# skipperro/selkies-gstreamer

Hardware: AMD Instinct MI355X
Metric: encoded fps + glass-to-glass p50 ms at 1920x1080; concurrent 60fps sessions/node (higher is better)
Workload: dtype uint8 pixels / int32 integer transforms (bit-exact vs CPU reference); 1 GPU; model=H.264 Constrained Baseline CAVLC, striped stripes 64px, CRF 25, global_batch=8, seq_len=1, parallelism=session-parallel dp1 x 8 sessions/GPU, resolution=1920x1080, backend=hip, deblock=auto, me_full=True, upload_overlap=False, frames_in_flight=1, num_refs=1, numa_node_rank0=0

## Files before the change

csrc/kernels/h264_kernels.hip:

```cpp
#include "h264_gpu.h"
#include "../codec/color.h"
#include "../codec/h264_mb.h"
#include "../codec/h264_ep.h"

namespace sk {
namespace h264 {
namespace gpu {

__device__ __forceinline__ int lane_id() { return threadIdx.x & 63; }

__device__ __forceinline__ void wave_sync() {
    __builtin_amdgcn_fence(__ATOMIC_RELEASE, "wavefront");
    __builtin_amdgcn_wave_barrier();
    __builtin_amdgcn_fence(__ATOMIC_ACQUIRE, "wavefront");
}

__device__ __forceinline__ int wave_sum(int v) {
    v += __builtin_amdgcn_mov_dpp(v, 0xB1, 0xF, 0xF, false);
    v += __builtin_amdgcn_mov_dpp(v, 0x4E, 0xF, 0xF, false);
    v += __builtin_amdgcn_mov_dpp(v, 0x124, 0xF, 0xF, false);
    v += __builtin_amdgcn_mov_dpp(v, 0x128, 0xF, 0xF, false);
    return __builtin_amdgcn_readlane(v, 0) + __builtin_amdgcn_readlane(v, 16) +
           __builtin_amdgcn_readlane(v, 32) + __builtin_amdgcn_readlane(v, 48);
}
// ... 212 lines not shown
            const uint4 a0 = *reinterpret_cast<const uint4*>(r0 + 4 * x0);
            const uint4 a1 = *reinterpret_cast<const uint4*>(r0 + 4 * x0 + 16);
            const uint4 b0 = *reinterpret_cast<const uint4*>(r1 + 4 * x0);
            const uint4 b1 = *reinterpret_cast<const uint4*>(r1 + 4 * x0 + 16);
            p0[0] = a0.x; p0[1] = a0.y; p0[2] = a0.z; p0[3] = a0.w;
            p0[4] = a1.x; p0[5] = a1.y; p0[6] = a1.z; p0[7] = a1.w;
            p1[0] = b0.x; p1[1] = b0.y; p1[2] = b0.z; p1[3] = b0.w;
            p1[4] = b1.x; p1[5] = b1.y; p1[6] = b1.z; p1[7] = b1.w;
        } else {
#pragma unroll
            for (int i = 0; i < 8; i++) {
                p0[i] = bgrx_px(r0, x0 + i, a.W);
                p1[i] = bgrx_px(r1, x0 + i, a.W);
            }
        }
        {
            const OverlayParams o0 = a.ov[0], o1 = a.ov[1];
            if (o0.on | o1.on) {
                const OverlayParams op[kOverlaySlots] = {o0, o1};
#pragma unroll
                for (int i = 0; i < 8; i++) {
                    const int x = sk_min(x0 + i, a.W - 1);
                    p0[i] = overlay_px(p0[i], x, y0, op, a.ov_img);
                    p1[i] = overlay_px(p1[i], x, y1, op, a.ov_img);
                }
            }
        }
        uint32_t ya[2] = {0, 0}, yb[2] = {0, 0}, cbw = 0, crw = 0;
#pragma unroll
        for (int q = 0; q < 4; q++) {
            uint8_t y[4], cb, cr;
            bgrx_quad_to_yuv((const uint8_t*)&p0[2 * q], (const uint8_t*)&p0[2 * q + 1], (const uint8_t*)&p1[2 * q],
                             (const uint8_t*)&p1[2 * q + 1], a.full_range, y, &cb, &cr);
            const int sh = 16 * (q & 1);
            ya[q >> 1] |= (uint32_t)(y[0] | (y[1] << 8)) << sh;
            yb[q >> 1] |= (uint32_t)(y[2] | (y[3] << 8)) << sh;
            cbw |= (uint32_t)cb << (8 * q);
            crw |= (uint32_t)cr << (8 * q);
        }
        const size_t oy = (size_t)(2 * qy) * a.stride_y + x0;
        const size_t oc = (size_t)qy * a.stride_c + x0 / 2;
        const uint2 pa = *reinterpret_cast<const uint2*>(a.prev.y + oy);
        const uint2 pb = *reinterpret_cast<const uint2*>(a.prev.y + oy + a.stride_y);
        const uint32_t pu = *reinterpret_cast<const uint32_t*>(a.prev.u + oc);
        const uint32_t pv = *reinterpret_cast<const uint32_t*>(a.prev.v + oc);
        diff = (pa.x != ya[0]) | (pa.y != ya[1]) | (pb.x != yb[0]) | (pb.y != yb[1]) | (pu != cbw) | (pv != crw);
        *reinterpret_cast<uint2*>(a.src.y + oy) = make_uint2(ya[0], ya[1]);
        *reinterpret_cast<uint2*>(a.src.y + oy + a.stride_y) = make_uint2(yb[0], yb[1]);
        *reinterpret_cast<uint32_t*>(a.src.u + oc) = cbw;
        *reinterpret_cast<uint32_t*>(a.src.v + oc) = crw;
    }
    if (diff || a.plan_ctl[1] == 0) mbd[item >> 1] = 1;
    __syncthreads();
    if (t < 16) {
        const int mbx = mbx0 + t;
        if (mbx < a.mb_w) a.mb_dirty[mby * a.mb_w + mbx] = (uint8_t)mbd[t];
    }
    if (__syncthreads_or(t < 16 && mbd[t] && mbx0 + t < a.mb_w) && t == 0)
        a.stripe_dirty[mby / a.rows_per_slice] = 1;
    host_words_store(a, host_words);
}

__global__ __launch_bounds__(256) void k_yuv_damage(FrameArgs a) {
    __shared__ int mbd[16];
    const int t = threadIdx.x;
    const int host_words = host_words_load(a);
    if (t < 16) mbd[t] = 0;
    __syncthreads();
    const int item = t & 31, qr = t >> 5;
    const int mby = blockIdx.y, mbx0 = blockIdx.x * 16;
    const int x0 = mbx0 * 16 + item * 8;
    const int qy = mby * 8 + qr;
    bool diff = false;
    if (x0 < a.stride_y) {
        const int W = a.W, H = a.H, cw = (W + 1) >> 1, ch = (H + 1) >> 1;
        const uint8_t* py = a.yuv;
        const uint8_t* pc = a.yuv + (size_t)W * H;
        const int y0 = min(2 * qy, H - 1), y1 = min(2 * qy + 1, H - 1), cy = min(qy, ch - 1);
        uint32_t ya[2] = {0, 0}, yb[2] = {0, 0}, cbw = 0, crw = 0;
#pragma unroll
        for (int i = 0; i < 8; i++) {
            const int x = min(x0 + i, W - 1);
            ya[i >> 2] |= (uint32_t)py[(size_t)y0 * W + x] << (8 * (i & 3));
            yb[i >> 2] |= (uint32_t)py[(size_t)y1 * W + x] << (8 * (i & 3));
        }
#pragma unroll
        for (int q = 0; q < 4; q++) {
            const int cx = min((x0 >> 1) + q, cw - 1);
            uint32_t u, v;
            if (a.yuv_fmt == 2) {
                const uint8_t* r = pc + (size_t)cy * (2 * cw) + 2 * cx;
                u = r[0];
                v = r[1];
            } else {
                u = pc[(size_t)cy * cw + cx];
                v = pc[(size_t)cw * ch + (size_t)cy * cw + cx];
            }
            cbw |= u << (8 * q);
            crw |= v << (8 * q);
        }
        const size_t oy = (size_t)(2 * qy) * a.stride_y + x0;
        const size_t oc = (size_t)qy * a.stride_c + x0 / 2;
        const uint2 pa = *reinterpret_cast<const uint2*>(a.prev.y + oy);
        const uint2 pb = *reinterpret_cast<const uint2*>(a.prev.y + oy + a.stride_y);
        const uint32_t pu = *reinterpret_cast<const uint32_t*>(a.prev.u + oc);
        const uint32_t pv = *reinterpret_cast<const uint32_t*>(a.prev.v + oc);
        diff = (pa.x != ya[0]) | (pa.y != ya[1]) | (pb.x != yb[0]) | (pb.y != yb[1]) | (pu != cbw) | (pv != crw);
        *reinterpret_cast<uint2*>(a.src.y + oy) = make_uint2(ya[0], ya[1]);
        *reinterpret_cast<uint2*>(a.src.y + oy + a.stride_y) = make_uint2(yb[0], yb[1]);
        *reinterpret_cast<uint32_t*>(a.src.u + oc) = cbw;
        *reinterpret_cast<uint32_t*>(a.src.v + oc) = crw;
    }
    if (diff || a.plan_ctl[1] == 0) mbd[item >> 1] = 1;
    __syncthreads();
    if (t < 16) {
        const int mbx = mbx0 + t;
        if (mbx < a.mb_w) a.mb_dirty[mby * a.mb_w + mbx] = (uint8_t)mbd[t];
    }
    if (__syncthreads_or(t < 16 && mbd[t] && mbx0 + t < a.mb_w) && t == 0)
        a.stripe_dirty[mby / a.rows_per_slice] = 1;
    host_words_store(a, host_words);
}

__device__ __forceinline__ uint32_t load_ref4(const uint8_t* row, int x, int stride) {
    if (x >= 0 && x + 3 <= stride - 1) {
        int xa = x & ~3, sh = x & 3;
        uint32_t w0 = *reinterpret_cast<const uint32_t*>(row + xa);
        if (sh == 0) return w0;
        uint32_t w1 = *reinterpret_cast<const uint32_t*>(row + xa + 4);
        return __builtin_amdgcn_alignbyte(w1, w0, sh);
    }
    uint32_t v = 0;
#pragma unroll
    for (int i = 0; i < 4; i++) v |= (uint32_t)row[sk_clip(x + i, 0, stride - 1)] << (8 * i);
    return v;
}

__device__ __forceinline__ uint32_t me_sad_lane(const FrameArgs& a, const uint8_t* refy, uint32_t sw, int mbx,
                                                int mby, int dx, int dy, int ylo, int yhi) {
    int l = lane_id();
    int row = l >> 2, col4 = (l & 3) * 4;
    int sy = sk_clip(mby * 16 + row + dy, ylo, yhi);
    uint32_t rw = load_ref4(refy + (size_t)sy * a.stride_y, mbx * 16 + col4 + dx, a.stride_y);
    return __builtin_amdgcn_sad_u8(sw, rw, 0u);
}

__device__ __forceinline__ int me_sad(const FrameArgs& a, const uint8_t* refy, uint32_t sw, int mbx,
                                      int mby, int dx, int dy, int ylo, int yhi) {
    return wave_sum((int)me_sad_lane(a, refy, sw, mbx, mby, dx, dy, ylo, yhi));
}

constexpr int kWin = 8;
constexpr int kWinWords = 10;
constexpr int kFsWinWords = kFsWin / 4 + 1;

struct MeWin {
    const uint32_t* w;
    int stride;
    int rad;
    int cx, cy;
    __device__ __forceinline__ bool has(int dx, int dy) const {
        return dx - cx >= -rad && dx - cx <= rad && dy - cy >= -rad && dy - cy <= rad;
    }
};

__device__ __forceinline__ uint32_t win_sad_lane(const MeWin& wn, uint32_t sw, int dx, int dy) {
    const int l = lane_id();
    const int row = l >> 2, col4 = (l & 3) * 4;
    const int bc = col4 + dx - wn.cx + wn.rad;
    const uint32_t* w = wn.w + (row + dy - wn.cy + wn.rad) * wn.stride + (bc >> 2);
    const int sh = bc & 3;
    const uint32_t rw = sh ? __builtin_amdgcn_alignbyte(w[1], w[0], sh) : w[0];
    return __builtin_amdgcn_sad_u8(sw, rw, 0u);
}

__device__ __forceinline__ int mb_activity(uint32_t sw) {
    const int psum = (int)(sw & 255) + (int)((sw >> 8) & 255) + (int)((sw >> 16) & 255) + (int)(sw >> 24);
    const int mean = (wave_sum(psum) + 128) >> 8;
    int dev = 0;
#pragma unroll
    for (int i = 0; i < 4; i++) dev += sk_abs((int)((sw >> (8 * i)) & 255) - mean);
    return wave_sum(dev);
}

__device__ __forceinline__ void me_search_mb(const FrameArgs& a, const SliceTask& t, const uint8_t* refy, int idx, int mbx,
                                             int mby, uint32_t sw, bool have_fs, int fsx, int fsy, uint32_t* win,
                                             bool big) {
    const int l = lane_id();
    if (t.action == ACT_I) {
        const int dev = mb_activity(sw);
        if (l == 0) a.me[idx] = MeResult{0, 0, 0, dev, 0, 0, 0};
        return;
    }
    const int ylo = t.pic_row0 * 16, yhi = (t.pic_row0 + t.pic_rows) * 16 - 1;
    const int lam = lambda_for_qp(rc_me_qp(*a.rc, t.qp));
    const int R = a.me_range;
    MeWin wn{win, big ? kFsWinWords : kWinWords, big ? kFsR : -1, 0, 0};
    auto sad_lane = [&](int dx, int dy) {
        return wn.has(dx, dy) ? win_sad_lane(wn, sw, dx, dy) : me_sad_lane(a, refy, sw, mbx, mby, dx, dy, ylo, yhi);
    };
    int cx[7], cy[7];
    bool ok[7];
    auto slot = [&](int k, bool valid, int ox, int oy) {
        const int j = valid ? oy * a.mb_w + ox : idx;
        ok[k] = valid;
        cx[k] = sk_clip(a.mvfield[2 * j], -R, R);
        cy[k] = sk_clip(a.mvfield[2 * j + 1], -R, R);
    };
    cx[0] = 0; cy[0] = 0; ok[0] = true;
    slot(1, true, mbx, mby);
    slot(2, mbx > 0, mbx - 1, mby);
    slot(3, mbx + 1 < a.mb_w, mbx + 1, mby);
    slot(4, mby - 1 >= t.pic_row0, mbx, mby - 1);
    slot(5, mby + 1 < t.pic_row0 + t.pic_rows, mbx, mby + 1);
    ok[6] = have_fs;
    cx[6] = sk_clip(fsx, -R, R);
    cy[6] = sk_clip(fsy, -R, R);
    int sd[8];
    {
        uint32_t p[8];
#pragma unroll
        for (int k = 0; k < 7; k++) p[k] = ok[k] ? sad_lane(cx[k], cy[k]) : 0u;
        p[7] = 0u;
#pragma unroll
        for (int k = 0; k < 8; k += 2) {
            const uint32_t s2 = (uint32_t)wave_sum((int)(p[k] | (p[k + 1] << 16)));
            sd[k] = (int)(s2 & 0xffff);
            sd[k + 1] = (int)(s2 >> 16);
        }
    }
    int bx = 0, by = 0;
    int bsad = sd[0];
    int bcost = bsad + lam * (sk_se_bits(0) + sk_se_bits(0));
#pragma unroll
    for (int k = 1; k < 7; k++) {
        if (!ok[k]) continue;
        int c = sd[k] + lam * (sk_se_bits(4 * cx[k]) + sk_se_bits(4 * cy[k]));
        if (c < bcost) { bcost = c; bx = cx[k]; by = cy[k]; bsad = sd[k]; }
    }
    if (!(big && wn.has(bx, by))) {
        wave_sync();
        const int r = l >> 1, h = l & 1;
        const int y = sk_clip(mby * 16 + by - kWin + r, ylo, yhi);
        const uint8_t* rowp = refy + (size_t)y * a.stride_y;
        const int x0 = mbx * 16 + bx - kWin + 16 * h;
#pragma unroll
        for (int k = 0; k < 5; k++) win[r * kWinWords + 4 * h + k] = load_ref4(rowp, x0 + 4 * k, a.stride_y);
        wn = MeWin{win, kWinWords, kWin, bx, by};
        wave_sync();
    }
    const int ddx[4] = {0, -1, 1, 0}, ddy[4] = {-1, 0, 0, 1};
    for (int it = 0; it < a.me_iters; it++) {
        uint32_t p[4];
        bool in_r[4];
#pragma unroll
        for (int k = 0; k < 4; k++) {
            const int x = bx + ddx[k], y = by + ddy[k];
            in_r[k] = !(x < -R || x > R || y < -R || y > R);
            p[k] = in_r[k] ? sad_lane(x, y) : 0u;
        }
        const uint32_t s01 = (uint32_t)wave_sum((int)(p[0] | (p[1] << 16)));
        const uint32_t s23 = (uint32_t)wave_sum((int)(p[2] | (p[3] << 16)));
        const int sds[4] = {(int)(s01 & 0xffff), (int)(s01 >> 16), (int)(s23 & 0xffff), (int)(s23 >> 16)};
        int nb = -1, ncost = bcost, nsad = 0;
#pragma unroll
        for (int k = 0; k < 4; k++) {
            if (!in_r[k]) continue;
            int x = bx + ddx[k], y = by + ddy[k];
            int c = sds[k] + lam * (sk_se_bits(4 * x) + sk_se_bits(4 * y));
            if (c < ncost) { ncost = c; nb = k; nsad = sds[k]; }
        }
        if (nb < 0) break;
        bx += ddx[nb]; by += ddy[nb]; bcost = ncost; bsad = nsad;
    }
    const int dev = mb_activity(sw);
    int refi = 0;
    if (t.num_refs > 1 && a.mb_dirty[idx]) {
        const int s1 = me_sad(a, ref1_planes(a, mby / a.rows_per_slice).y, sw, mbx, mby, 0, 0, ylo, yhi);
        if (s1 + 3 * lam < bcost) {
            bx = by = 0;
            bsad = s1;
            refi = 1;
        }
    }
    if (l == 0) {
        MeResult r;
        r.mvx = (int16_t)bx;
        r.mvy = (int16_t)by;
        r.sad = bsad;
        r.intra_est = dev;
        r.ref = (int16_t)refi;
        r.fx = r.fy = 0;
        a.me[idx] = r;
    }
}

__global__ __launch_bounds__(64) void k_motion_search(FrameArgs a) {
    __shared__ uint32_t win[32 * kWinWords];
    int nmb = a.mb_w * a.mb_h;
    int idx = xcd_remap(blockIdx.x, gridDim.x);
    if (idx >= nmb) return;
    int mbx = idx % a.mb_w, mby = idx / a.mb_w;
    const SliceTask t = a.tasks[mby / a.rows_per_slice];
    if (t.action != ACT_P && t.action != ACT_I) return;
    int l = lane_id();
    uint32_t sw = *reinterpret_cast<const uint32_t*>(a.src.y + (size_t)(mby * 16 + (l >> 2)) * a.stride_y +
                                                     mbx * 16 + (l & 3) * 4);
    const bool have_fs = a.me_full && t.action == ACT_P && a.mb_dirty[idx];
    const int fsx = have_fs ? a.fs_mv[2 * idx] : 0, fsy = have_fs ? a.fs_mv[2 * idx + 1] : 0;
    me_search_mb(a, t, ref0_planes(a, mby / a.rows_per_slice).y, idx, mbx, mby, sw, have_fs, fsx, fsy, win, false);
}

typedef int v4i __attribute__((ext_vector_type(4)));

constexpr int kFsBlkWords = 5;
constexpr int kFsSqInts = 2 * kFsR + 4;

__device__ __forceinline__ uint64_t fs_search(const FrameArgs& a, const uint8_t* refy, uint32_t* win, uint32_t* blk, int* sq,
                                              int mbx, int mby, uint32_t sw, int ylo, int yhi) {
    constexpr int WW = kFsWin / 4;
    constexpr int WP = kFsWinWords;
    constexpr int BP = kFsBlkWords;
    constexpr int SP = kFsSqInts;
    const int l = lane_id();
    for (int i = l; i < kFsWin * WW; i += 64) {
        const int wy = i / WW, q = i - wy * WW;
        const int y = sk_clip(mby * 16 - kFsR + wy, ylo, yhi);
        win[wy * WP + q] = load_ref4(refy + (size_t)y * a.stride_y, mbx * 16 - kFsR + 4 * q, a.stride_y);
    }
    blk[(l >> 2) * BP + (l & 3)] = sw;
    wave_sync();
    if (l < kFsWin) {
        uint32_t rw[WW];
#pragma unroll
        for (int q = 0; q < WW; q++) rw[q] = win[l * WP + q];
        int sqv[kFsWin];
#pragma unroll
        for (int c = 0; c < kFsWin; c++) {
            const int v = (int)((rw[c >> 2] >> (8 * (c & 3))) & 255) - 128;
            sqv[c] = v * v;
        }
        int acc = 0;
#pragma unroll
        for (int c = 0; c < 16; c++) acc += sqv[c];
        int out[2 * kFsR];
        out[0] = acc;
#pragma unroll
        for (int x = 1; x < 2 * kFsR; x++) {
            acc += sqv[x + 15] - sqv[x - 1];
            out[x] = acc;
        }
#pragma unroll
        for (int x = 0; x < 2 * kFsR; x += 4)
            *reinterpret_cast<int4*>(&sq[l * SP + x]) = make_int4(out[x], out[x + 1], out[x + 2], out[x + 3]);
    }
    wave_sync();
    if (l < 2 * kFsR) {
        int col[kFsWin];
#pragma unroll
        for (int r = 0; r < kFsWin; r++) col[r] = sq[r * SP + l];
        int acc = 0;
#pragma unroll
        for (int r = 0; r < 16; r++) acc += col[r];
#pragma unroll
        for (int dy = 0; dy < 2 * kFsR; dy++) {
            sq[dy * SP + l] = acc;
            acc += col[dy + 16] - col[dy];
        }
    }
    const int i16 = l & 15, g = l >> 4;
    v4i acc[2][2];
#pragma unroll
    for (int mt = 0; mt < 2; mt++)
#pragma unroll
        for (int nt = 0; nt < 2; nt++) acc[mt][nt] = v4i{0, 0, 0, 0};
#pragma unroll
    for (int ks = 0; ks < kFsWin / 4; ks++) {
        const int rr = 4 * ks + g;
        v4i bf[2];
#pragma unroll
        for (int nt = 0; nt < 2; nt++) {
            const int src = rr - (16 * nt + i16);
            const bool in = src >= 0 && src < 16;
#pragma unroll
            for (int q = 0; q < 4; q++) bf[nt][q] = in ? (int)(blk[(in ? src : 0) * BP + q] ^ 0x80808080u) : 0;
        }
#pragma unroll
        for (int mt = 0; mt < 2; mt++) {
            const int b0 = 16 * mt + i16;
            const uint32_t* wr = win + rr * WP + (b0 >> 2);
            const int sh = b0 & 3;
            uint32_t w5[5];
#pragma unroll
            for (int q = 0; q < 5; q++) w5[q] = wr[q];
            v4i af;
#pragma unroll
            for (int q = 0; q < 4; q++) af[q] = (int)(__builtin_amdgcn_alignbyte(w5[q + 1], w5[q], sh) ^ 0x80808080u);
#pragma unroll
            for (int nt = 0; nt < 2; nt++)
                if (ks >= 4 * nt && ks <= 4 * nt + 7)
                    acc[mt][nt] = __builtin_amdgcn_mfma_i32_16x16x64_i8(af, bf[nt], acc[mt][nt], 0, 0, 0);
        }
    }
    wave_sync();
    uint64_t best = ~0ull;
#pragma unroll
    for (int mt = 0; mt < 2; mt++)
#pragma unroll
        for (int nt = 0; nt < 2; nt++) {
            const int dyw = 16 * nt + i16;
            const int4 sv = *reinterpret_cast<const int4*>(&sq[dyw * SP + 16 * mt + 4 * g]);
            const int svr[4] = {sv.x, sv.y, sv.z, sv.w};
#pragma unroll
            for (int reg = 0; reg < 4; reg++) {
                const int dxw = 16 * mt + 4 * g + reg;
                const uint64_t k = fs_key(svr[reg] - 2 * acc[mt][nt][reg], dyw, dxw);
                best = k < best ? k : best;
            }
        }
#pragma unroll
    for (int o = 1; o < 64; o <<= 1) {
        const uint64_t other = __shfl_xor(best, o);
        best = other < best ? other : best;
    }
    return best;
}

__global__ __launch_bounds__(256) void k_me(FrameArgs a) {
    __shared__ uint32_t win_s[4][kFsWin * kFsWinWords];
    __shared__ uint32_t blk_s[4][16 * kFsBlkWords];
    __shared__ __align__(16) int sq_s[4][kFsWin * kFsSqInts];
    static_assert(kFsWin * kFsWinWords >= 32 * kWinWords, "the small window lives in the wave's win_s region");
    const int w = threadIdx.x >> 6, l = lane_id();
    const int nmb = a.mb_w * a.mb_h;
    const int idx = xcd_remap(blockIdx.x, gridDim.x) * 4 + w;
    if (idx >= nmb) return;
    const int mbx = idx % a.mb_w, mby = idx / a.mb_w;
    const SliceTask t = a.tasks[mby / a.rows_per_slice];
    if (t.action != ACT_P && t.action != ACT_I) return;
    const uint8_t* refy = ref0_planes(a, mby / a.rows_per_slice).y;
    const uint32_t sw = *reinterpret_cast<const uint32_t*>(a.src.y + (size_t)(mby * 16 + (l >> 2)) * a.stride_y +
                                                           mbx * 16 + (l & 3) * 4);
    bool have_fs = false, big = false;
    int fsx = 0, fsy = 0;
    if (t.action == ACT_P && a.mb_dirty[idx]) {
        have_fs = true;
        const int ylo = t.pic_row0 * 16, yhi = (t.pic_row0 + t.pic_rows) * 16 - 1;
        const int R = a.me_range;
        const int px = sk_clip(a.mvfield[2 * idx], -R, R), py = sk_clip(a.mvfield[2 * idx + 1], -R, R);
        if (me_sad(a, refy, sw, mbx, mby, px, py, ylo, yhi) == 0) {
            fsx = px;
            fsy = py;
        } else {
            const uint64_t best = fs_search(a, refy, win_s[w], blk_s[w], sq_s[w], mbx, mby, sw, ylo, yhi);
            fsx = __builtin_amdgcn_readfirstlane(fs_key_dx(best));
            fsy = __builtin_amdgcn_readfirstlane(fs_key_dy(best));
            big = true;
        }
        if (l == 0) {
            a.fs_mv[2 * idx] = (int16_t)fsx;
            a.fs_mv[2 * idx + 1] = (int16_t)fsy;
        }
    }
    me_search_mb(a, t, refy, idx, mbx, mby, sw, have_fs, fsx, fsy, win_s[w], big);
}

__global__ __launch_bounds__(256) void k_plan(FrameArgs a) {
    const int ns = a.num_slices, tid = threadIdx.x;
    StripeState* st = a.plan_state;
    StripeState& pic = st[ns];
    if (a.plan_ctl[1] == 1) {
        if (a.fullframe) {
            bool idr = true;
            for (int s = tid; s < ns; s += 256) idr &= a.tasks[s].final_action == ACT_I && a.tasks[s].idr_on_intra;
            idr = __syncthreads_and(idr);
            if (tid == 0) commit_picture(pic, idr, a.plan_cfg.num_refs);
            if (a.ltr_excl && tid == 0)
                ltr::ltr_commit_rps(a.ltr_slots, a.ltr_state[ns], idr, a.tasks[0].frame_num, a.mb_w * a.mb_h, 0, ns,
                                    a.ltr_task);
            else if (a.ltr_slots && tid == 0)
                ltr::ltr_commit(a.ltr_slots, a.ltr_state[ns], true, idr, a.tasks[0].frame_num, a.mb_w * a.mb_h, 0, ns,
                                a.ltr_task);
        } else {
            if (a.ltr_slots)
                for (int s = tid; s < ns; s += 256) {
                    const SliceTask& t = a.tasks[s];
                    ltr::ltr_commit(a.ltr_slots, a.ltr_state[s], t.final_action != ACT_NONE,
                                    t.final_action == ACT_I && t.idr_on_intra, t.frame_num, t.num_rows * a.mb_w, s, s + 1,
                                    a.ltr_task);
                }
            for (int s = tid; s < ns; s += 256)
                commit_stripe(st[s], a.tasks[s].final_action, a.plan_cfg.num_refs, a.tasks[s].idr_on_intra != 0);
        }
    }
    __shared__ int hk[6];
    if (tid < 6) hk[tid] = a.key_dev[tid];
    __syncthreads();
    const int kq = hk[0];
    const bool key = kq != a.plan_ctl[0];
    __syncthreads();
    if (key) {
        for (int s = tid; s < ns; s += 256) st[s].need_idr = true;
        if (tid == 0) pic.need_idr = true;
    }
    __syncthreads();
    PlanConfig pc = a.plan_cfg;
    const int qo = hk[1];
    const int po = hk[2];
    if (qo > 0) pc.qp = qo;
    if (po > 0) pc.paint_qp = po;
    {
        const int mode = hk[5] != a.rc->seq ? hk[3] : a.rc->mode;
        if (mode == RC_CBR) pc.use_paint_over = 0;
    }
    for (int s = tid; s < ns; s += 256) {
        st[s].subpel_prev = st[s].subpel_hits;
        st[s].subpel_hits = 0;
        const int r0 = s * a.rows_per_slice, nr = min(a.rows_per_slice, a.mb_h - r0);
        plan_stripe(pc, st[s], pic, a.stripe_dirty[s] != 0, r0, nr, a.mb_h, a.tasks[s]);
        a.stripe_dirty[s] = 0;
    }
    __syncthreads();
    if (tid == 0) {
        a.plan_ctl[0] = kq;
        a.plan_ctl[1] = 1;
    }
}

__global__ __launch_bounds__(256) void k_ltr_match(FrameArgs a) {
    __shared__ int red[4];
    const int band = blockIdx.x, c = blockIdx.y, s = blockIdx.z, tid = threadIdx.x;
    const int ns = a.num_slices;
    const SliceTask t = a.tasks[s];
    const int s0 = a.fullframe ? 0 : s, s1 = a.fullframe ? ns : s + 1;
    const int mb0 = (a.fullframe ? 0 : t.first_row) * a.mb_w, n = (a.fullframe ? a.mb_h : t.num_rows) * a.mb_w;
    int nd = 0, key = 0, anyp = 0;
    for (int i = tid; i < n; i += 256) nd += a.mb_dirty[mb0 + i] != 0;
    for (int i = s0 + tid; i < s1; i += 256) {
        key |= a.tasks[i].action == ACT_I;
        anyp |= a.tasks[i].action == ACT_P;
    }
    nd = wave_sum(nd);
    if (lane_id() == 0) red[tid >> 6] = nd;
    key = __syncthreads_or(key);
    anyp = __syncthreads_or(anyp);
    nd = red[0] + red[1] + red[2] + red[3];
    const int valid = a.ltr_state[a.fullframe ? ns : s].valid;
    const bool gate = anyp && !key && ltr::ltr_large(nd, n) && valid != 0;
    if (band == 0 && c == 0 && tid == 0) {
        a.ltr_cnt[2 * s] = nd;
        a.ltr_cnt[2 * s + 1] = gate;
    }
    if (!gate || t.action != ACT_P || band >= t.num_rows || (c > 0 && !((valid >> (c - 1)) & 1))) return;
    const uint8_t* ref = c ? a.ltr.y + (size_t)(c - 1) * a.ltr_ny : a.ref.y;
    const size_t o = (size_t)(t.first_row + band) * 16 * a.stride_y;
    const uint4* q = reinterpret_cast<const uint4*>(a.src.y + o);
    const uint4* r = reinterpret_cast<const uint4*>(ref + o);
    uint32_t sum = 0;
    for (int i = tid; i < a.stride_y; i += 256) {
        const uint4 x = q[i], y = r[i];
        sum = __builtin_amdgcn_sad_u8(x.x, y.x, sum);
        sum = __builtin_amdgcn_sad_u8(x.y, y.y, sum);
        sum = __builtin_amdgcn_sad_u8(x.z, y.z, sum);
        sum = __builtin_amdgcn_sad_u8(x.w, y.w, sum);
    }
    sum = (uint32_t)wave_sum((int)sum);
    __syncthreads();
    if (lane_id() == 0) red[tid >> 6] = (int)sum;
    __syncthreads();
    if (tid == 0)
        a.ltr_part[((size_t)s * ltr::kLtrSadCols + c) * a.rows_per_slice + band] =
            (uint32_t)red[0] + (uint32_t)red[1] + (uint32_t)red[2] + (uint32_t)red[3];
}

__global__ __launch_bounds__(256) void k_ltr_decide(FrameArgs a) {
    const int ns = a.num_slices, tid = threadIdx.x;
    for (int i = tid; i < ns * ltr::kLtrSadCols; i += 256) {
        const int s = i / ltr::kLtrSadCols, c = i - s * ltr::kLtrSadCols;
        const int valid = a.ltr_state[a.fullframe ? ns : s].valid;
        uint32_t sum = 0;
        if (a.ltr_cnt[2 * s + 1] && a.tasks[s].action == ACT_P && c <= a.ltr_slots && (c == 0 || ((valid >> (c - 1)) & 1)))
            for (int b = 0; b < a.tasks[s].num_rows; b++) sum += a.ltr_part[(size_t)i * a.rows_per_slice + b];
        a.ltr_sad[i] = sum;
    }
    __syncthreads();
    const int streams = a.fullframe ? 1 : ns;
    for (int k = tid; k < streams; k += 256) {
        const int s0 = a.fullframe ? 0 : k, s1 = a.fullframe ? ns : k + 1;
        bool key = false, anyp = false;
        int rows = 0;
        for (int s = s0; s < s1; s++) {
            key |= a.tasks[s].action == ACT_I;
            anyp |= a.tasks[s].action == ACT_P;
            rows += a.tasks[s].num_rows;
        }
        if (a.ltr_excl) ltr::ltr_expire(a.ltr_slots, a.ltr_state[ns], a.tasks[s0].frame_num, a.ltr_max_age);
        ltr::ltr_decide(a.ltr_slots, a.ltr_state[a.fullframe ? ns : k], a.ltr_cnt[2 * s0], rows * a.mb_w, anyp && !key,
                        a.tasks[s0].frame_num, kFrameNumMask, s0, s1,
                        [&](int s) { return a.tasks[s].action == ACT_P; }, a.ltr_sad, a.ltr_task);
        for (int s = s0; s < s1; s++)
            if (a.ltr_task[s].slot >= 0 && !a.ltr_excl) a.tasks[s].num_refs = 2;
    }
}

__global__ __launch_bounds__(256) void k_decide(FrameArgs a) {
    __shared__ long long red[2][4];
    const int s = blockIdx.x;
    SliceTask& t = a.tasks[s];
    const bool planned_p = t.action == ACT_P;
    const bool p = planned_p && t.allow_scenecut;
    __shared__ int red1[4];
    long long sad = 0, dev = 0;
    int ref1 = 0;
    if (planned_p || t.action == ACT_I) {
        const int first = t.first_row * a.mb_w, nmb = t.num_rows * a.mb_w;
        for (int i = threadIdx.x; i < nmb; i += 256) {
            const MeResult r = a.me[first + i];
// ... 2080 lines not shown
            w[2 + (le >> 1)] |= (uint32_t)bh << sh;
            w[10] |= (bv ? 1u << le : 0u) | (bh ? 16u << le : 0u);
        }
    const int qc = cur.qpy, cc = H264_CHROMA_QP[qc];
    w[4] = db_pack_par((left.qpy + qc + 1) >> 1);
    w[5] = db_pack_par((top.qpy + qc + 1) >> 1);
    w[6] = db_pack_par(qc);
    w[7] = db_pack_par((H264_CHROMA_QP[left.qpy] + cc + 1) >> 1);
    w[8] = db_pack_par((H264_CHROMA_QP[top.qpy] + cc + 1) >> 1);
    w[9] = db_pack_par(cc);
    uint4* o = a.dbe + 3 * (size_t)idx;
    o[0] = make_uint4(w[0], w[1], w[2], w[3]);
    o[1] = make_uint4(w[4], w[5], w[6], w[7]);
    o[2] = make_uint4(w[8], w[9], w[10], 0);
}

template <int MAXR>
__global__ __launch_bounds__(64 * MAXR) void k_deblock(FrameArgs a) {
    constexpr int kSlots = 8;
    __shared__ uint32_t ring[MAXR][kSlots][32][4];
    __shared__ uint4 erec[MAXR][kSlots][3];
    const SliceTask t = a.tasks[blockIdx.x];
    if (t.final_action != ACT_P && t.final_action != ACT_I) return;
    if (!slice_deblock(a.deblock, t)) return;
    const int r = threadIdx.x >> 6, l = lane_id();
    const int R = t.num_rows, W = a.mb_w;
    const int mby = t.first_row + r;
    const bool band = r < R;
    const bool act = l < 32, chroma = l >= 16;
    const int li = chroma ? (l & 7) : (l & 15);
    const int nrows = chroma ? 8 : 16;
    const int lbase = chroma ? 16 + (l & 8) : 0;
    const int ldw = chroma ? 1 : 3;
    const int bsh = 4 * (chroma ? li >> 1 : li >> 2);
    const uint8_t* src = chroma ? ((l & 8) ? a.rec.v : a.rec.u) : a.rec.y;
    uint8_t* dst = chroma ? ((l & 8) ? a.ref.v : a.ref.u) : a.ref.y;
    const int mbyc = sk_min(mby, t.first_row + R - 1);
    const size_t rowoff = chroma ? (size_t)(mbyc * 8 + li) * a.stride_c : (size_t)(mbyc * 16 + li) * a.stride_y;
    const int mbbytes = chroma ? 8 : 16;

    const int half2 = chroma ? 0 : 8;
    auto load_px = [&](int x) {
        const uint8_t* p0 = src + rowoff + sk_clip(x, 0, W - 1) * mbbytes;
        const uint2 lo = *reinterpret_cast<const uint2*>(p0), hi = *reinterpret_cast<const uint2*>(p0 + half2);
        return make_uint4(lo.x, lo.y, hi.x, hi.y);
    };
    auto load_rec = [&](int x) {
        return a.dbe[3 * ((size_t)mbyc * W + sk_clip(x, 0, W - 1)) + sk_min(sk_max(l - 32, 0), 2)];
    };

    int x = -1 - 2 * r;
    uint4 pre = make_uint4(0, 0, 0, 0);
    if (band) pre = act ? load_px(x + 1) : load_rec(x + 1);
    const int steps = W + 2 * R + 2;
    for (int k = 0; k < steps; k++, x++) {
        if (band) {
            if (x + 1 >= 0 && x + 1 < W) {
                const int sn = (x + 1) & (kSlots - 1);
                if (act) *reinterpret_cast<uint4*>(ring[r][sn][l]) = pre;
                else if (l < 35) erec[r][sn][l - 32] = pre;
            }
            pre = act ? load_px(x + 2) : load_rec(x + 2);
            wave_sync();

            if (x >= 0 && x < W) {
                const int sl = x & (kSlots - 1);
                const uint4 e0 = erec[r][sl][0], e1 = erec[r][sl][1], e2 = erec[r][sl][2];
                const uint32_t emask = e2.z | ((e2.z & 0x44u) >> 1);
                auto bs_of = [&](uint32_t w01, uint32_t w23, int e) -> int {
                    if (chroma) {
                        if (e >= 2) return 0;
                        return __builtin_amdgcn_ubfe(e == 0 ? w01 : w23, bsh, 4);
                    }
                    return __builtin_amdgcn_ubfe(e < 2 ? w01 : w23, 16 * (e & 1) + bsh, 4);
                };
                const uint32_t p_left = chroma ? e1.w : e1.x, p_top = chroma ? e2.x : e1.y;
                const uint32_t p_in = chroma ? e2.y : e1.z;
                uint32_t* own = ring[r][sl][0];
                if (emask & 15u) {
                    uint32_t* lp = ring[r][(x - 1) & (kSlots - 1)][act ? l : 0];
                    uint32_t* op = own + 4 * (act ? l : 0);
                    int v[20];
                    unpack4((emask & 1u) ? lp[ldw] : 0u, v);
#pragma unroll
                    for (int q = 0; q < 4; q++) unpack4(op[q], v + 4 + 4 * q);
#pragma unroll
                    for (int e = 0; e < 4; e++)
                        if (emask & (1u << e)) {
                            const int bs = act ? bs_of(e0.x, e0.y, e) : 0;
                            if (e == 0) db_filter_line<true>(v, bs, p_left, chroma);
                            else db_filter_line<false>(v + 4 * e, bs, p_in, chroma);
                        }
                    if (act) {
                        if (emask & 1u) lp[ldw] = pack4(v);
#pragma unroll
                        for (int q = 0; q < 4; q++) op[q] = pack4(v + 4 + 4 * q);
                    }
                    wave_sync();
                }
                if (emask & 0xF0u) {
                    uint8_t* ob = reinterpret_cast<uint8_t*>(own) + lbase * 16 + li;
                    uint8_t* tb = reinterpret_cast<uint8_t*>(ring[sk_max(r - 1, 0)][sl][0]) +
                                  (lbase + nrows - 4) * 16 + li;
                    const bool top_on = (emask & 16u) && act;
                    int v[20];
#pragma unroll
                    for (int q = 0; q < 4; q++) v[q] = top_on ? tb[q * 16] : 0;
#pragma unroll
                    for (int q = 0; q < 16; q++) v[4 + q] = act ? ob[sk_min(q, nrows - 1) * 16] : 0;
#pragma unroll
                    for (int e = 0; e < 4; e++)
                        if (emask & (16u << e)) {
                            const int bs = act ? bs_of(e0.z, e0.w, e) : 0;
                            if (e == 0) db_filter_line<true>(v, bs, p_top, chroma);
                            else db_filter_line<false>(v + 4 * e, bs, p_in, chroma);
                        }
                    if (act) {
                        if (top_on) {
#pragma unroll
                            for (int q = 1; q < 4; q++) tb[q * 16] = (uint8_t)v[q];
                        }
#pragma unroll
                        for (int q = 0; q < 16; q++)
                            if (q < nrows) ob[q * 16] = (uint8_t)v[4 + q];
                    }
                    wave_sync();
                }
            }
            const int xb = x - 3;
            if (act && xb >= 0 && xb < W) {
                const uint4 q = *reinterpret_cast<const uint4*>(ring[r][xb & (kSlots - 1)][l]);
                uint8_t* p0 = dst + rowoff + xb * mbbytes;
                *reinterpret_cast<uint2*>(p0) = make_uint2(q.x, q.y);
                *reinterpret_cast<uint2*>(p0 + half2) = chroma ? make_uint2(q.x, q.y) : make_uint2(q.z, q.w);
            }
        }
        lds_barrier();
    }
}

void launch_convert_damage(const FrameArgs& a, hipStream_t s) {
    dim3 grid((a.mb_w + 15) / 16, a.mb_h);
    if (a.yuv_fmt) hipLaunchKernelGGL(k_yuv_damage, grid, dim3(256), 0, s, a);
    else hipLaunchKernelGGL(k_convert_damage, grid, dim3(256), 0, s, a);
}

void launch_frontend(const FrameArgs& a, hipStream_t s) {
    int nmb = a.mb_w * a.mb_h;
    hipLaunchKernelGGL(k_plan, dim3(1), dim3(256), 0, s, a);
    if (a.ltr_slots) {
        hipLaunchKernelGGL(k_ltr_match, dim3(a.rows_per_slice, 1 + a.ltr_slots, a.num_slices), dim3(256), 0, s, a);
        hipLaunchKernelGGL(k_ltr_decide, dim3(1), dim3(256), 0, s, a);
    }
    if (a.me_full) hipLaunchKernelGGL(k_me, dim3((nmb + 3) / 4), dim3(256), 0, s, a);
    else hipLaunchKernelGGL(k_motion_search, dim3(nmb), dim3(64), 0, s, a);
    hipLaunchKernelGGL(k_decide, dim3(a.num_slices), dim3(256), 0, s, a);
    hipLaunchKernelGGL(k_rc_qp, dim3(1), dim3(64), 0, s, a);
    if (a.subpel) hipLaunchKernelGGL(k_subpel, dim3((nmb + 3) / 4), dim3(256), 0, s, a);
}

void launch_rc_guard_sizes(const FrameArgs& a, const int* sizes, int n, int* redo, bool chained, hipStream_t s) {
    hipLaunchKernelGGL(k_rc_guard_sizes, dim3(1), dim3(256), 0, s, a, sizes, n, redo, chained ? 1 : 0);
}

void launch_rc_account(const FrameArgs& a, const int* sizes, int n, int stride, int per_slice, hipStream_t s) {
    hipLaunchKernelGGL(k_rc_account, dim3(1), dim3(64), 0, s, a, sizes, n, stride, per_slice);
}

static void launch_code(const FrameArgs& a, hipStream_t s) {
    int nmb = a.mb_w * a.mb_h;
    hipLaunchKernelGGL(k_code_inter, dim3((nmb + 3) / 4), dim3(256), 0, s, a);
    hipLaunchKernelGGL(k_intra_prep, dim3((nmb + 3) / 4), dim3(256), 0, s, a);
    if (a.nal_per_slice > 1)
        hipLaunchKernelGGL(k_code_intra_sub, dim3((a.num_slices * a.nal_per_slice + 3) / 4), dim3(256), 0, s, a);
    else if (a.rows_per_slice <= 4)
        hipLaunchKernelGGL(k_code_intra<4>, dim3(a.num_slices), dim3(64 * 5), 0, s, a);
    else
        hipLaunchKernelGGL(k_code_intra<kMaxRows - 1>, dim3(a.num_slices), dim3(64 * kMaxRows), 0, s, a);
    hipLaunchKernelGGL(k_cavlc, dim3((nmb + 3) / 4), dim3(256), 0, s, a);
}

void launch_encode(const FrameArgs& a, hipStream_t s, bool guard) {
    int nmb = a.mb_w * a.mb_h;
    launch_frontend(a, s);
    if (a.aq_strength > 0) hipLaunchKernelGGL(k_aq, dim3((nmb + 3) / 4), dim3(256), 0, s, a);
    launch_code(a, s);
    if (guard && a.rc_redo) {
        hipLaunchKernelGGL(k_slice_pack<true>, dim3(a.num_slices), dim3(kPackThreads), 0, s, a);
        hipLaunchKernelGGL(k_rc_guard, dim3(1), dim3(256), 0, s, a);
        FrameArgs b = a;
        b.gate = a.rc_redo;
        launch_code(b, s);
    }
    hipLaunchKernelGGL(k_slice_pack<false>, dim3(a.num_slices), dim3(kPackThreads), 0, s, a);
}

void launch_commit(const FrameArgs& a, hipStream_t s, bool filter, bool account) {
    hipLaunchKernelGGL(k_commit, dim3((a.mb_w + 15) / 16, a.mb_h), dim3(256), 0, s, a, account ? 1 : 0);
    if (a.deblock && filter) {
        const int nmb = a.mb_w * a.mb_h;
        hipLaunchKernelGGL(k_deblock_prep, dim3((nmb + 3) / 4), dim3(256), 0, s, a);
        hipLaunchKernelGGL(k_deblock_edges, dim3((nmb + 255) / 256), dim3(256), 0, s, a);
        if (a.rows_per_slice <= 4)
            hipLaunchKernelGGL(k_deblock<4>, dim3(a.num_slices), dim3(64 * a.rows_per_slice), 0, s, a);
        else
            hipLaunchKernelGGL(k_deblock<kMaxRows>, dim3(a.num_slices), dim3(64 * a.rows_per_slice), 0, s, a);
    }
}

}
}
}
```

Baseline: 5907 frames/s (1920x1080 H.264, all sessions, all GPUs).

## Share full-search reference window across four horizontally adjacent macroblocks in k_me

```diff
diff --git a/csrc/kernels/h264_kernels.hip b/csrc/kernels/h264_kernels.hip
--- a/csrc/kernels/h264_kernels.hip
+++ b/csrc/kernels/h264_kernels.hip
@@ -388,13 +388,16 @@
 
 constexpr int kWin = 8;
 constexpr int kWinWords = 10;
-constexpr int kFsWinWords = kFsWin / 4 + 1;
+constexpr int kFsGroup = 4;
+constexpr int kFsWinBytes = kFsWin + 16 * (kFsGroup - 1);
+constexpr int kFsWinWords = kFsWinBytes / 4 + 1;
 
 struct MeWin {
     const uint32_t* w;
     int stride;
     int rad;
     int cx, cy;
+    uint32_t bias;
     __device__ __forceinline__ bool has(int dx, int dy) const {
         return dx - cx >= -rad && dx - cx <= rad && dy - cy >= -rad && dy - cy <= rad;
     }
@@ -407,7 +410,7 @@
     const uint32_t* w = wn.w + (row + dy - wn.cy + wn.rad) * wn.stride + (bc >> 2);
     const int sh = bc & 3;
     const uint32_t rw = sh ? __builtin_amdgcn_alignbyte(w[1], w[0], sh) : w[0];
-    return __builtin_amdgcn_sad_u8(sw, rw, 0u);
+    return __builtin_amdgcn_sad_u8(sw, rw ^ wn.bias, 0u);
 }
 
 __device__ __forceinline__ int mb_activity(uint32_t sw) {
@@ -421,7 +424,7 @@
 
 __device__ __forceinline__ void me_search_mb(const FrameArgs& a, const SliceTask& t, const uint8_t* refy, int idx, int mbx,
                                              int mby, uint32_t sw, bool have_fs, int fsx, int fsy, uint32_t* win,
-                                             bool big) {
+                                             const MeWin& bigw) {
     const int l = lane_id();
     if (t.action == ACT_I) {
         const int dev = mb_activity(sw);
@@ -431,7 +434,8 @@
     const int ylo = t.pic_row0 * 16, yhi = (t.pic_row0 + t.pic_rows) * 16 - 1;
     const int lam = lambda_for_qp(rc_me_qp(*a.rc, t.qp));
     const int R = a.me_range;
-    MeWin wn{win, big ? kFsWinWords : kWinWords, big ? kFsR : -1, 0, 0};
+    const bool big = bigw.rad >= 0;
+    MeWin wn = bigw;
     auto sad_lane = [&](int dx, int dy) {
         return wn.has(dx, dy) ? win_sad_lane(wn, sw, dx, dy) : me_sad_lane(a, refy, sw, mbx, mby, dx, dy, ylo, yhi);
     };
@@ -474,6 +478,7 @@
         int c = sd[k] + lam * (sk_se_bits(4 * cx[k]) + sk_se_bits(4 * cy[k]));
         if (c < bcost) { bcost = c; bx = cx[k]; by = cy[k]; bsad = sd[k]; }
     }
+    STAMP(63, 7);
     if (!(big && wn.has(bx, by))) {
         wave_sync();
         const int r = l >> 1, h = l & 1;
@@ -482,7 +487,7 @@
         const int x0 = mbx * 16 + bx - kWin + 16 * h;
 #pragma unroll
         for (int k = 0; k < 5; k++) win[r * kWinWords + 4 * h + k] = load_ref4(rowp, x0 + 4 * k, a.stride_y);
-        wn = MeWin{win, kWinWords, kWin, bx, by};
+        wn = MeWin{win, kWinWords, kWin, bx, by, 0u};
         wave_sync();
     }
     const int ddx[4] = {0, -1, 1, 0}, ddy[4] = {-1, 0, 0, 1};
@@ -509,6 +514,7 @@
         if (nb < 0) break;
         bx += ddx[nb]; by += ddy[nb]; bcost = ncost; bsad = nsad;
     }
+    STAMP(63, 8);
     const int dev = mb_activity(sw);
     int refi = 0;
     if (t.num_refs > 1 && a.mb_dirty[idx]) {
@@ -529,6 +535,7 @@
         r.fx = r.fy = 0;
         a.me[idx] = r;
     }
+    STAMP(63, 9);
 }
 
 __global__ __launch_bounds__(64) void k_motion_search(FrameArgs a) {
@@ -544,161 +551,181 @@
                                                      mbx * 16 + (l & 3) * 4);
     const bool have_fs = a.me_full && t.action == ACT_P && a.mb_dirty[idx];
     const int fsx = have_fs ? a.fs_mv[2 * idx] : 0, fsy = have_fs ? a.fs_mv[2 * idx + 1] : 0;
-    me_search_mb(a, t, ref0_planes(a, mby / a.rows_per_slice).y, idx, mbx, mby, sw, have_fs, fsx, fsy, win, false);
+    me_search_mb(a, t, ref0_planes(a, mby / a.rows_per_slice).y, idx, mbx, mby, sw, have_fs, fsx, fsy, win,
+                 MeWin{nullptr, 0, -1, 0, 0, 0u});
 }
 
 typedef int v4i __attribute__((ext_vector_type(4)));
 
-constexpr int kFsBlkWords = 5;
-constexpr int kFsSqInts = 2 * kFsR + 4;
+constexpr int kFsBlkRows = 15 + 16 + 16;
+constexpr int kFsCols = 2 * kFsR + 16 * (kFsGroup - 1);
+constexpr int kFsSqInts = kFsCols + 4;
+static_assert(kFsCols % kFsGroup == 0 && (kFsCols / kFsGroup) % 4 == 0, "row sums: one column run per wave, int4 stores");
 
 __device__ __forceinline__ uint64_t fs_search(const FrameArgs& a, const uint8_t* refy, uint32_t* win, uint32_t* blk, int* sq,
-                                              int mbx, int mby, uint32_t sw, int ylo, int yhi) {
-    constexpr int WW = kFsWin / 4;
+                                              int mbx0, int mby, uint32_t sw, bool search, int ylo, int yhi) {
+    constexpr int WW = kFsWinBytes / 4;
     constexpr int WP = kFsWinWords;
-    constexpr int BP = kFsBlkWords;
     constexpr int SP = kFsSqInts;
-    const int l = lane_id();
-    for (int i = l; i < kFsWin * WW; i += 64) {
+    constexpr int SEG = kFsCols / kFsGroup;
+    const int tid = threadIdx.x, w = tid >> 6, l = lane_id();
+    for (int i = tid; i < kFsWin * WW; i += 64 * kFsGroup) {
         const int wy = i / WW, q = i - wy * WW;
         const int y = sk_clip(mby * 16 - kFsR + wy, ylo, yhi);
-        win[wy * WP + q] = load_ref4(refy + (size_t)y * a.stride_y, mbx * 16 - kFsR + 4 * q, a.stride_y);
-    }
-    blk[(l >> 2) * BP + (l & 3)] = sw;
-    wave_sync();
+        win[wy * WP + q] = load_ref4(refy + (size_t)y * a.stride_y, mbx0 * 16 - kFsR + 4 * q, a.stride_y) ^ 0x80808080u;
+    }
+    if (search) {
+        if (l < 60) blk[l] = 0u;
+        blk[31 * 4 + l] = 0u;
+        blk[(15 + (l >> 2)) * 4 + (l & 3)] = sw ^ 0x80808080u;
+    }
+    __syncthreads();
+    STAMP(63, 2);
     if (l < kFsWin) {
-        uint32_t rw[WW];
-#pragma unroll
-        for (int q = 0; q < WW; q++) rw[q] = win[l * WP + q];
-        int sqv[kFsWin];
-#pragma unroll
-        for (int c = 0; c < kFsWin; c++) {
-            const int v = (int)((rw[c >> 2] >> (8 * (c & 3))) & 255) - 128;
+        constexpr int NB = SEG + 15;
+        uint32_t rw[(NB + 3) / 4];
+#pragma unroll
+        for (int q = 0; q < (NB + 3) / 4; q++) rw[q] = win[l * WP + (SEG / 4) * w + q];
+        int sqv[NB];
+#pragma unroll
+        for (int c = 0; c < NB; c++) {
+            const int v = (int)(int8_t)(rw[c >> 2] >> (8 * (c & 3)));
             sqv[c] = v * v;
         }
         int acc = 0;
 #pragma unroll
         for (int c = 0; c < 16; c++) acc += sqv[c];
-        int out[2 * kFsR];
+        int out[SEG];
         out[0] = acc;
 #pragma unroll
-        for (int x = 1; x < 2 * kFsR; x++) {
+        for (int x = 1; x < SEG; x++) {
             acc += sqv[x + 15] - sqv[x - 1];
             out[x] = acc;
         }
 #pragma unroll
-        for (int x = 0; x < 2 * kFsR; x += 4)
-            *reinterpret_cast<int4*>(&sq[l * SP + x]) = make_int4(out[x], out[x + 1], out[x + 2], out[x + 3]);
-    }
-    wave_sync();
-    if (l < 2 * kFsR) {
-        int col[kFsWin];
-#pragma unroll
-        for (int r = 0; r < kFsWin; r++) col[r] = sq[r * SP + l];
+        for (int x = 0; x < SEG; x += 4)
+            *reinterpret_cast<int4*>(&sq[l * SP + SEG * w + x]) = make_int4(out[x], out[x + 1], out[x + 2], out[x + 3]);
+    }
+    __syncthreads();
+    STAMP(63, 3);
+    if (tid < 2 * kFsCols) {
+        const int h = tid >= kFsCols, c = tid - h * kFsCols;
+        int col[31];
+#pragma unroll
+        for (int r = 0; r < 31; r++) col[r] = sq[(16 * h + r) * SP + c];
         int acc = 0;
 #pragma unroll
         for (int r = 0; r < 16; r++) acc += col[r];
 #pragma unroll
-        for (int dy = 0; dy < 2 * kFsR; dy++) {
-            sq[dy * SP + l] = acc;
-            acc += col[dy + 16] - col[dy];
-        }
-    }
+        for (int dy = 0; dy < 16; dy++) {
+            sq[(32 * h + dy) * SP + c] = acc;
+            if (dy < 15) acc += col[dy + 16] - col[dy];
+        }
+    }
+    STAMP(63, 4);
     const int i16 = l & 15, g = l >> 4;
     v4i acc[2][2];
 #pragma unroll
     for (int mt = 0; mt < 2; mt++)
 #pragma unroll
         for (int nt = 0; nt < 2; nt++) acc[mt][nt] = v4i{0, 0, 0, 0};
-#pragma unroll
-    for (int ks = 0; ks < kFsWin / 4; ks++) {
-        const int rr = 4 * ks + g;
-        v4i bf[2];
-#pragma unroll
-        for (int nt = 0; nt < 2; nt++) {
-            const int src = rr - (16 * nt + i16);
-            const bool in = src >= 0 && src < 16;
-#pragma unroll
-            for (int q = 0; q < 4; q++) bf[nt][q] = in ? (int)(blk[(in ? src : 0) * BP + q] ^ 0x80808080u) : 0;
-        }
-#pragma unroll
-        for (int mt = 0; mt < 2; mt++) {
-            const int b0 = 16 * mt + i16;
-            const uint32_t* wr = win + rr * WP + (b0 >> 2);
-            const int sh = b0 & 3;
-            uint32_t w5[5];
-#pragma unroll
-            for (int q = 0; q < 5; q++) w5[q] = wr[q];
-            v4i af;
-#pragma unroll
-            for (int q = 0; q < 4; q++) af[q] = (int)(__builtin_amdgcn_alignbyte(w5[q + 1], w5[q], sh) ^ 0x80808080u);
-#pragma unroll
-            for (int nt = 0; nt < 2; nt++)
-                if (ks >= 4 * nt && ks <= 4 * nt + 7)
-                    acc[mt][nt] = __builtin_amdgcn_mfma_i32_16x16x64_i8(af, bf[nt], acc[mt][nt], 0, 0, 0);
-        }
-    }
-    wave_sync();
+    if (search) {
+        v4i bf[8];
+#pragma unroll
+        for (int k = 0; k < 8; k++) bf[k] = *reinterpret_cast<const v4i*>(&blk[(4 * k + g - i16 + 15) * 4]);
+        const uint32_t* wr0 = win + 4 * w + (i16 >> 2);
+        const int sh = i16 & 3;
+#pragma unroll
+        for (int ks = 0; ks < kFsWin / 4; ks++) {
+            const uint32_t* wr = wr0 + (4 * ks + g) * WP;
+            uint32_t w9[9];
+#pragma unroll
+            for (int q = 0; q < 9; q++) w9[q] = wr[q];
+#pragma unroll
+            for (int mt = 0; mt < 2; mt++) {
+                v4i af;
+#pragma unroll
+                for (int q = 0; q < 4; q++) af[q] = (int)__builtin_amdgcn_alignbyte(w9[4 * mt + q + 1], w9[4 * mt + q], sh);
+#pragma unroll
+                for (int nt = 0; nt < 2; nt++)
+                    if (ks >= 4 * nt && ks <= 4 * nt + 7)
+                        acc[mt][nt] = __builtin_amdgcn_mfma_i32_16x16x64_i8(af, bf[ks - 4 * nt], acc[mt][nt], 0, 0, 0);
+            }
+        }
+    }
+    STAMP(63, 5);
+    __syncthreads();
     uint64_t best = ~0ull;
-#pragma unroll
-    for (int mt = 0; mt < 2; mt++)
-#pragma unroll
-        for (int nt = 0; nt < 2; nt++) {
-            const int dyw = 16 * nt + i16;
-            const int4 sv = *reinterpret_cast<const int4*>(&sq[dyw * SP + 16 * mt + 4 * g]);
-            const int svr[4] = {sv.x, sv.y, sv.z, sv.w};
-#pragma unroll
-            for (int reg = 0; reg < 4; reg++) {
-                const int dxw = 16 * mt + 4 * g + reg;
-                const uint64_t k = fs_key(svr[reg] - 2 * acc[mt][nt][reg], dyw, dxw);
-                best = k < best ? k : best;
-            }
-        }
-#pragma unroll
-    for (int o = 1; o < 64; o <<= 1) {
-        const uint64_t other = __shfl_xor(best, o);
-        best = other < best ? other : best;
-    }
+    if (search) {
+#pragma unroll
+        for (int mt = 0; mt < 2; mt++)
+#pragma unroll
+            for (int nt = 0; nt < 2; nt++) {
+                const int dyw = 16 * nt + i16;
+                const int4 sv = *reinterpret_cast<const int4*>(&sq[(32 * nt + i16) * SP + 16 * w + 16 * mt + 4 * g]);
+                const int svr[4] = {sv.x, sv.y, sv.z, sv.w};
+#pragma unroll
+                for (int reg = 0; reg < 4; reg++) {
+                    const int dxw = 16 * mt + 4 * g + reg;
+                    const uint64_t k = fs_key(svr[reg] - 2 * acc[mt][nt][reg], dyw, dxw);
+                    best = k < best ? k : best;
+                }
+            }
+#pragma unroll
+        for (int o = 1; o < 64; o <<= 1) {
+            const uint64_t other = __shfl_xor(best, o);
+            best = other < best ? other : best;
+        }
+    }
+    STAMP(63, 6);
     return best;
 }
 
 __global__ __launch_bounds__(256) void k_me(FrameArgs a) {
-    __shared__ uint32_t win_s[4][kFsWin * kFsWinWords];
-    __shared__ uint32_t blk_s[4][16 * kFsBlkWords];
-    __shared__ __align__(16) int sq_s[4][kFsWin * kFsSqInts];
-    static_assert(kFsWin * kFsWinWords >= 32 * kWinWords, "the small window lives in the wave's win_s region");
+    __shared__ uint32_t win_s[kFsWin * kFsWinWords];
+    __shared__ __align__(16) int sq_s[kFsWin * kFsSqInts];
+    __shared__ __align__(16) uint32_t small_s[kFsGroup][32 * kWinWords];
+    static_assert(32 * kWinWords >= kFsBlkRows * 4 && (32 * kWinWords) % 4 == 0, "the block lives in the wave's small window");
     const int w = threadIdx.x >> 6, l = lane_id();
-    const int nmb = a.mb_w * a.mb_h;
-    const int idx = xcd_remap(blockIdx.x, gridDim.x) * 4 + w;
-    if (idx >= nmb) return;
-    const int mbx = idx % a.mb_w, mby = idx / a.mb_w;
+    const int gw = (a.mb_w + kFsGroup - 1) / kFsGroup;
+    const int b = xcd_remap(blockIdx.x, gridDim.x);
+    const int mby = b / gw, mbx0 = (b - mby * gw) * kFsGroup, mbx = mbx0 + w;
+    if (mby >= a.mb_h) return;
     const SliceTask t = a.tasks[mby / a.rows_per_slice];
     if (t.action != ACT_P && t.action != ACT_I) return;
+    STAMP(63, 0);
+    const bool valid = mbx < a.mb_w;
+    const int idx = mby * a.mb_w + mbx;
     const uint8_t* refy = ref0_planes(a, mby / a.rows_per_slice).y;
-    const uint32_t sw = *reinterpret_cast<const uint32_t*>(a.src.y + (size_t)(mby * 16 + (l >> 2)) * a.stride_y +
-                                                           mbx * 16 + (l & 3) * 4);
-    bool have_fs = false, big = false;
+    const uint32_t sw = valid ? *reinterpret_cast<const uint32_t*>(a.src.y + (size_t)(mby * 16 + (l >> 2)) * a.stride_y +
+                                                                   mbx * 16 + (l & 3) * 4)
+                              : 0u;
+    const int ylo = t.pic_row0 * 16, yhi = (t.pic_row0 + t.pic_rows) * 16 - 1;
+    bool have_fs = false, search = false;
     int fsx = 0, fsy = 0;
-    if (t.action == ACT_P && a.mb_dirty[idx]) {
+    if (valid && t.action == ACT_P && a.mb_dirty[idx]) {
         have_fs = true;
-        const int ylo = t.pic_row0 * 16, yhi = (t.pic_row0 + t.pic_rows) * 16 - 1;
         const int R = a.me_range;
-        const int px = sk_clip(a.mvfield[2 * idx], -R, R), py = sk_clip(a.mvfield[2 * idx + 1], -R, R);
-        if (me_sad(a, refy, sw, mbx, mby, px, py, ylo, yhi) == 0) {
-            fsx = px;
-            fsy = py;
-        } else {
-            const uint64_t best = fs_search(a, refy, win_s[w], blk_s[w], sq_s[w], mbx, mby, sw, ylo, yhi);
+        fsx = sk_clip(a.mvfield[2 * idx], -R, R);
+        fsy = sk_clip(a.mvfield[2 * idx + 1], -R, R);
+        search = me_sad(a, refy, sw, mbx, mby, fsx, fsy, ylo, yhi) != 0;
+    }
+    const bool any = __syncthreads_or(search);
+    STAMP(63, 1);
+    if (any) {
+        const uint64_t best = fs_search(a, refy, win_s, small_s[w], sq_s, mbx0, mby, sw, search, ylo, yhi);
+        if (search) {
             fsx = __builtin_amdgcn_readfirstlane(fs_key_dx(best));
             fsy = __builtin_amdgcn_readfirstlane(fs_key_dy(best));
-            big = true;
-        }
-        if (l == 0) {
-            a.fs_mv[2 * idx] = (int16_t)fsx;
-            a.fs_mv[2 * idx + 1] = (int16_t)fsy;
-        }
-    }
-    me_search_mb(a, t, refy, idx, mbx, mby, sw, have_fs, fsx, fsy, win_s[w], big);
+        }
+    }
+    if (!valid) return;
+    if (have_fs && l == 0) {
+        a.fs_mv[2 * idx] = (int16_t)fsx;
+        a.fs_mv[2 * idx + 1] = (int16_t)fsy;
+    }
+    me_search_mb(a, t, refy, idx, mbx, mby, sw, have_fs, fsx, fsy, small_s[w],
+                 MeWin{win_s + 4 * w, kFsWinWords, search ? kFsR : -1, 0, 0, 0x80808080u});
 }
 
 __global__ __launch_bounds__(256) void k_plan(FrameArgs a) {
@@ -3085,7 +3112,7 @@
         hipLaunchKernelGGL(k_ltr_match, dim3(a.rows_per_slice, 1 + a.ltr_slots, a.num_slices), dim3(256), 0, s, a);
         hipLaunchKernelGGL(k_ltr_decide, dim3(1), dim3(256), 0, s, a);
     }
-    if (a.me_full) hipLaunchKernelGGL(k_me, dim3((nmb + 3) / 4), dim3(256), 0, s, a);
+    if (a.me_full) hipLaunchKernelGGL(k_me, dim3(a.mb_h * ((a.mb_w + kFsGroup - 1) / kFsGroup)), dim3(256), 0, s, a);
     else hipLaunchKernelGGL(k_motion_search, dim3(nmb), dim3(64), 0, s, a);
     hipLaunchKernelGGL(k_decide, dim3(a.num_slices), dim3(256), 0, s, a);
     hipLaunchKernelGGL(k_rc_qp, dim3(1), dim3(64), 0, s, a);
```

Measured after the change: 6008 frames/s (1920x1080 H.264, all sessions, all GPUs) (median of 6 runs). +1.7%, better.
